# IanYeung/RealVSR

Measured on AMD Instinct MI355X. Metric: HR frames/sec (fwd+bwd) on 5-frame 180x320 LR windows, higher is better.
Workload: dtype f32 (bf16x3 GEMM); 1 GPU; EDVR-M nf64, 5-frame 180x320 LR windows, batch 8 per GPU, x4 output, VideoSRModel.optimize_parameters: fwd + LapPyr(ssim,cb) on Y + GWLoss on CbCr + bwd + Adam step; per_gpu_batch=8, global_batch=8, parallelism=sequence-dp1, gemm=bf16x3 (3-term bf16 split on v_mfma_f32_32x32x16_bf16, f32 accumulate), lf_term=ssim (restated IQA_pytorch.SSIM, parity unpinned)

## Files before the change

realvsr_amd/csrc/conv2_kernels.hip:

```cpp
#define RVSR_DEFINE_PACK
#include "conv_plan.h"

#include "bf16x3.h"

#ifdef RVSR_ABL5
constexpr int ABL5 = RVSR_ABL5;
#else
constexpr int ABL5 = 0;
#endif

#ifdef RVSR_TIMELINE
__device__ unsigned long long rvsr_dbg[512];
extern "C" int rvsr_debug_read(unsigned long long* out) { return (int)hipMemcpyFromSymbol(out, HIP_SYMBOL(rvsr_dbg), sizeof(unsigned long long) * 512); }
#define STAMP(i) do { if (blockIdx.x == 77 && tid == 0) rvsr_dbg[(i)] = __builtin_amdgcn_s_memtime(); } while (0)
#else
#define STAMP(i) do {} while (0)
#endif

template <int MT, int MODE>
__device__ __forceinline__ void conv2_epilogue(f32x16 (&acc)[MT][2], const ConvFwdParams& p, const float* bias_s, int b,
                                               int o0, int row0, int col, int hi) {
    const float neg = p.act == 0 ? 1.f : (p.act == 1 ? 0.f : p.slope);
    const bool col_ok = col < p.Wout;
    const size_t HW = (size_t)p.Hout * p.Wout;
#pragma unroll
    for (int n = 0; n < 2; ++n) {
        const int row = row0 + n;
        if (row >= p.Hout) continue;
        const size_t pix = (size_t)row * p.Wout + col;
#pragma unroll
        for (int m = 0; m < MT; ++m) {
            float resv[16];
            if (MODE == 1) {
#pragma unroll
                for (int r = 0; r < 16; ++r) {
                    const int o = o0 + m * 32 + 4 * hi + (r & 3) + 8 * (r >> 2);
                    const bool ok = col_ok && o < p.Co;
                    resv[r] = p.res[ok ? ((size_t)b * p.Co + o) * HW + pix : 0];
                }
            }
#pragma unroll
            for (int r = 0; r < 16; ++r) {
                const int ol = m * 32 + 4 * hi + (r & 3) + 8 * (r >> 2);
                const int o = o0 + ol;
                const bool ok = col_ok && o < p.Co;
                const int oc = ok ? o : 0;
                float v = acc[m][n][r] + bias_s[ol];
                v = v > 0.f ? v : v * neg;
                if (MODE == 3) {
                    const size_t idx = (((size_t)b * (p.Co >> 2) + (oc >> 2)) * (2 * p.Hout) + 2 * row + ((oc >> 1) & 1)) *
                                           (2 * p.Wout) + 2 * col + (oc & 1);
                    if (ok) p.out1[idx] = v;
                } else if (MODE == 2) {
                    const bool first = oc < p.Co1;
                    float* dst = first ? p.out1 : p.out2;
                    const size_t idx = ((size_t)b * (first ? p.Co1 : p.Co - p.Co1) + (first ? oc : oc - p.Co1)) * HW + pix;
                    if (ok) dst[idx] = v;
                } else {
                    if (MODE == 1) v += resv[r];
                    if (ok) p.out1[((size_t)b * p.Co + oc) * HW + pix] = v;
                }
            }
        }
    }
}

template <int MT, int MODE>
__device__ __forceinline__ void conv2_epilogue_v4(f32x16 (&acc)[MT][2], const ConvFwdParams& p, const float* bias_s, int b,
                                                  int o0, int row0, int x0, int lo, int hi) {
    const float neg = p.act == 0 ? 1.f : (p.act == 1 ? 0.f : p.slope);
    const int j = lo & 3, col4 = x0 + (lo & ~3);
    const bool col_ok = col4 < p.Wout;
    const unsigned HW = (unsigned)(p.Hout * p.Wout), HW4 = 4u * HW;
    const __amdgpu_buffer_rsrc_t out_rs = buf_view_2g(p.out1 + (size_t)b * p.Co * HW);
    const __amdgpu_buffer_rsrc_t res_rs = buf_view_2g(MODE == 1 ? p.res + (size_t)b * p.Co * HW : p.out1);
#pragma unroll
    for (int n = 0; n < 2; ++n) {
        const int row = row0 + n;
        if (row >= p.Hout) continue;
        const unsigned lane_off = 4u * ((unsigned)(4 * hi + j) * HW + (unsigned)row * p.Wout + col4);
#pragma unroll
        for (int m = 0; m < MT; ++m) {
            float4 resv[4];
            unsigned off[4];
#pragma unroll
            for (int rg = 0; rg < 4; ++rg) {
                const int ob = o0 + m * 32 + 8 * rg;
                off[rg] = col_ok && ob + 4 * hi + j < p.Co ? lane_off : 0x80000000u;
                if (MODE == 1) {
                    typedef float f32x4v __attribute__((ext_vector_type(4)));
                    const f32x4v q = __builtin_bit_cast(f32x4v, __builtin_amdgcn_raw_buffer_load_b128(res_rs, (int)(off[rg] + (unsigned)ob * HW4), 0, 0));
                    resv[rg] = make_float4(q.x, q.y, q.z, q.w);
                }
            }
#pragma unroll
            for (int rg = 0; rg < 4; ++rg) {
                float r0 = acc[m][n][4 * rg + 0], r1 = acc[m][n][4 * rg + 1], r2 = acc[m][n][4 * rg + 2], r3 = acc[m][n][4 * rg + 3];
                quad_transpose4(r0, r1, r2, r3, lo);
                const int ol = m * 32 + 8 * rg + 4 * hi + j;
                const float bb = bias_s[ol];
                float4 v = make_float4(r0 + bb, r1 + bb, r2 + bb, r3 + bb);
                v.x = v.x > 0.f ? v.x : v.x * neg; v.y = v.y > 0.f ? v.y : v.y * neg;
                v.z = v.z > 0.f ? v.z : v.z * neg; v.w = v.w > 0.f ? v.w : v.w * neg;
                if (MODE == 1) { v.x += resv[rg].x; v.y += resv[rg].y; v.z += resv[rg].z; v.w += resv[rg].w; }
                buf_store4(out_rs, off[rg] + (unsigned)(o0 + m * 32 + 8 * rg) * HW4, 0u, v);
            }
        }
    }
}

__device__ __forceinline__ void half_swap(float& a, float& b) {
    asm volatile("s_nop 1\n\tv_permlane32_swap_b32 %0, %1\n\ts_nop 0" : "+v"(a), "+v"(b));
}
template <int MT, int MODE>
__device__ __forceinline__ void conv2_epilogue_wide(f32x16 (&acc)[MT][2], const ConvFwdParams& p, const float* bias_s, int b,
                                                    int o0, int row, int x0, int lo, int hi) {
    if (row >= p.Hout) return;
    const float neg = (p.act == 0 || MODE == 4) ? 1.f : (p.act == 1 ? 0.f : p.slope);
    const int lane = 32 * hi + lo, jn = lane >> 4, Gn = lane & 15;
    const int src4 = 4 * (4 * Gn + jn);
    const int col4 = x0 + 4 * Gn;
    const bool col_ok = col4 < p.Wout;
    const unsigned HW = (unsigned)(p.Hout * p.Wout), HW4 = 4u * HW;
    const __amdgpu_buffer_rsrc_t out_rs = buf_view_2g(p.out1 + (size_t)b * p.Co * HW);
    const __amdgpu_buffer_rsrc_t res_rs = buf_view_2g(MODE == 1 || MODE == 4 ? p.res + (size_t)b * p.Co * HW : p.out1);
    const unsigned lane_off = 4u * ((unsigned)jn * HW + (unsigned)row * p.Wout + col4);
    const int j = lo & 3;
#pragma unroll
    for (int m = 0; m < MT; ++m) {
#pragma unroll
        for (int rg = 0; rg < 4; ++rg) {
            float4 resv[2];
            unsigned off[2];
#pragma unroll
            for (int s = 0; s < 2; ++s) {
                const int ob = o0 + m * 32 + 8 * rg + 4 * s;
                off[s] = col_ok && ob + jn < p.Co ? lane_off : 0x80000000u;
                if (MODE == 1 || MODE == 4) {
                    typedef float f32x4v __attribute__((ext_vector_type(4)));
                    const f32x4v q = __builtin_bit_cast(f32x4v, __builtin_amdgcn_raw_buffer_load_b128(res_rs, (int)(off[s] + (unsigned)ob * HW4), 0, 0));
                    resv[s] = make_float4(q.x, q.y, q.z, q.w);
                }
            }
            float r[2][4];
            const float bb = bias_s[m * 32 + 8 * rg + 4 * hi + j];
#pragma unroll
            for (int n = 0; n < 2; ++n) {
                r[n][0] = acc[m][n][4 * rg + 0]; r[n][1] = acc[m][n][4 * rg + 1]; r[n][2] = acc[m][n][4 * rg + 2]; r[n][3] = acc[m][n][4 * rg + 3];
                quad_transpose4(r[n][0], r[n][1], r[n][2], r[n][3], lo);
#pragma unroll
                for (int e = 0; e < 4; ++e) {
                    const float v = r[n][e] + bb;
                    r[n][e] = v > 0.f ? v : v * neg;
                }
            }
#pragma unroll
            for (int e = 0; e < 4; ++e) half_swap(r[0][e], r[1][e]);
#pragma unroll
            for (int s = 0; s < 2; ++s)
#pragma unroll
                for (int e = 0; e < 4; ++e)
                    r[s][e] = __builtin_bit_cast(float, __builtin_amdgcn_ds_bpermute(src4, __builtin_bit_cast(int, r[s][e])));
#pragma unroll
            for (int s = 0; s < 2; ++s) {
                float4 v = make_float4(r[s][0], r[s][1], r[s][2], r[s][3]);
                if (MODE == 1) { v.x += resv[s].x; v.y += resv[s].y; v.z += resv[s].z; v.w += resv[s].w; }
                if (MODE == 4) {
                    v.x *= resv[s].x > 0.f ? 1.f : p.slope; v.y *= resv[s].y > 0.f ? 1.f : p.slope;
                    v.z *= resv[s].z > 0.f ? 1.f : p.slope; v.w *= resv[s].w > 0.f ? 1.f : p.slope;
                }
                if (!(ABL5 & 2) || (m == 0 && rg == 0 && s == 0))
                buf_store4(out_rs, off[s] + (unsigned)(o0 + m * 32 + 8 * rg + 4 * s) * HW4, 0u, v);
            }
        }
    }
}

template <int KS, int STRIDE, int MT, int CCG, bool ACT_IN, int NW>
__global__ __launch_bounds__(NW * 64, 2) void conv_fwd2_kernel(const ConvFwdParams p) {
    constexpr int T = KS * KS, PAD = KS / 2, TH = 2 * NW, TW = 32, NTHR = NW * 64;
    constexpr int IH = (TH - 1) * STRIDE + KS, IW = (TW - 1) * STRIDE + KS;
    constexpr int MP = MT * 32, NOCT = 2 * CCG, NPOS = IH * IW;
    constexpr int WVEC = T * NOCT * MP;
    extern __shared__ __attribute__((aligned(16))) unsigned char smem_raw[];
    bf16x8* xs_hi = reinterpret_cast<bf16x8*>(smem_raw);
    bf16x8* xs_lo = xs_hi + NOCT * NPOS;
    bf16x8* ws_hi = xs_lo + NOCT * NPOS;
    bf16x8* ws_lo = ws_hi + WVEC;
    float* bias_s = reinterpret_cast<float*>(ws_lo + WVEC);
    const int tid = threadIdx.x, lane = tid & 63, wave = tid >> 6, lo = lane & 31, hi = lane >> 5;
    const TView& va = p.in.a;
    const TView& vb = p.in.b;
    const int C1 = va.C, Ctot = va.C + vb.C;
    const int nchunks = (Ctot + 16 * CCG - 1) / (16 * CCG);

    const unsigned nmb = (p.Co + MP - 1) / MP, nty = (p.Hout + TH - 1) / TH, ntx = (p.Wout + TW - 1) / TW;
    const unsigned items = ntx * nty * nmb * p.B;
    const unsigned xcd = blockIdx.x & 7, wq = blockIdx.x >> 3, nwq = (gridDim.x + 7 - xcd) >> 3;
    const unsigned q8 = items >> 3, r8 = items & 7;
    const unsigned range0 = xcd < r8 ? xcd * (q8 + 1) : r8 * (q8 + 1) + (xcd - r8) * q8;
    const unsigned range1 = range0 + q8 + (xcd < r8 ? 1 : 0);

    int x0 = 0, y0 = 0, mb = 0, b = 0;
    auto decode = [&](unsigned S) {
        const unsigned t = S % (p.ntx * nty);
        x0 = (int)(t % p.ntx) * TW;
        y0 = (int)(t / p.ntx) * TH;
        mb = (int)((S / (p.ntx * nty)) % nmb);
        b = (int)(S / (p.ntx * nty * nmb));
    };

    constexpr int NIT = (NOCT * NPOS + NTHR - 1) / NTHR;
    constexpr int NWV = (2 * WVEC + NTHR - 1) / NTHR;
    float vin[NIT][8];
    float ain[ACT_IN ? NIT : 1][8];
    int nvalid[NIT];

    __amdgpu_buffer_rsrc_t xa_rs = buf_view_2g(va.p), xb_rs = buf_view_2g(va.p), act_rs = buf_view_2g(va.p);
    auto tile_views = [&]() {
        if (va.mode != 0) return;
        const size_t hw = (size_t)va.Hs * va.Ws;
        xa_rs = buf_view_2g(va.p + (size_t)b * va.C * hw);
        if (vb.C) xb_rs = buf_view_2g(vb.p + (size_t)b * vb.C * hw);
        if (ACT_IN) act_rs = buf_view_2g(va.act + (size_t)b * va.C * hw);
    };
    auto issue_loads = [&](int chunk, int i_lo = 0, int i_hi = 1 << 20) {
        const int c0 = chunk * 16 * CCG;
#pragma unroll
        for (int i = 0; i < NIT; ++i) {
            if (i < i_lo || i >= i_hi) continue;
            const int it_raw = tid + i * NTHR;
            const bool live = it_raw < NOCT * NPOS;
            const int it = live ? it_raw : 0;
            const int oc = it / NPOS, pos = it - oc * NPOS;
            const int r = pos / IW, s = pos - r * IW;
            const int gy = y0 * STRIDE - PAD + r, gx = x0 * STRIDE - PAD + s;
            const int cb = c0 + oc * 8;
            const bool inb = live && gy >= 0 && gx >= 0 && gy < va.Hv && gx < va.Wv && cb < Ctot;
            const int gyc = gy < 0 ? 0 : (gy >= va.Hv ? va.Hv - 1 : gy), gxc = gx < 0 ? 0 : (gx >= va.Wv ? va.Wv - 1 : gx);
            if (va.mode == 0) {
                const bool second = c0 >= C1;
                const int Cb = second ? vb.C : va.C, cl0 = second ? c0 - C1 : c0;
                const unsigned hw4 = 4u * (unsigned)(va.Hs * va.Ws);
                const bool pos_ok = live && gy >= 0 && gx >= 0 && gy < va.Hv && gx < va.Wv;
                const unsigned vo = pos_ok ? 4u * (unsigned)(gy * va.Ws + gx) + (unsigned)(8 * oc) * hw4 : 0x80000000u;
                const int lane_nch = Cb - cl0 - 8 * oc;
                nvalid[i] = 8;
#pragma unroll
                for (int j = 0; j < 8; ++j) {
                    const unsigned vo_j = j < lane_nch ? vo : 0x80000000u;
                    const unsigned so = (unsigned)(cl0 + j) * hw4;
                    vin[i][j] = buf_load(second ? xb_rs : xa_rs, vo_j, so);
                    if (ACT_IN) ain[i][j] = buf_load(act_rs, vo_j, so);
                }
            } else {
                const size_t hw = (size_t)va.Hs * va.Ws;
                const int cbc = inb ? cb : 0;
                const size_t base = ((size_t)b * (va.C >> 2) + (cbc >> 2)) * hw + (size_t)(2 * gyc) * va.Ws + 2 * gxc;
                nvalid[i] = inb ? 8 : 0;
#pragma unroll
                for (int j = 0; j < 8; ++j) {
                    const size_t idx = base + (j >> 2) * hw + ((j >> 1) & 1) * va.Ws + (j & 1);
                    vin[i][j] = va.p[idx];
                    if (ACT_IN) ain[i][j] = va.act[idx];
                }
            }
        }
    };
    auto commit_inputs = [&](int i_lo = 0, int i_hi = 1 << 20) {
#pragma unroll
        for (int i = 0; i < NIT; ++i) {
            if (i < i_lo || i >= i_hi) continue;
            const int it = tid + i * NTHR;
            float v[8];
#pragma unroll
            for (int j = 0; j < 8; ++j) {
                float x = ACT_IN ? vin[i][j] * (ain[i][j] > 0.f ? 1.f : va.slope) : vin[i][j];
                v[j] = j < nvalid[i] ? x : 0.f;
            }
            bf16x8 h8, l8;
            split8(v, h8, l8);
            if (it < NOCT * NPOS) {
                xs_hi[it] = h8;
                xs_lo[it] = l8;
            }
        }
    };
    auto commit_to_lds = [&](int chunk, bool inputs_done = false) {
        const bf16x8* src = reinterpret_cast<const bf16x8*>(p.wpack) + ((size_t)mb * nchunks + chunk) * 2 * WVEC;
        constexpr int WB = MT >= 4 ? 3 : 9;
        constexpr bool OVERLAP = !ACT_IN && MT <= 2;
        if (!OVERLAP && !inputs_done) commit_inputs();
#pragma unroll
        for (int base = 0; base < NWV; base += WB) {
            bf16x8 wv[WB];
#pragma unroll
            for (int i = 0; i < WB; ++i) {
                const int e = tid + (base + i) * NTHR;
                wv[i] = src[(base + i < NWV && e < 2 * WVEC) ? e : 0];
            }
            if (OVERLAP && base == 0 && !inputs_done) commit_inputs();
#pragma unroll
            for (int i = 0; i < WB; ++i) {
                const int e = tid + (base + i) * NTHR;
                if (base + i < NWV && e < 2 * WVEC) ws_hi[e] = wv[i];
            }
        }
        if (chunk == 0 && tid < MP) {
            const int o = mb * MP + tid;
            bias_s[tid] = (p.bias != nullptr && o < p.Co) ? p.bias[o] : 0.f;
        }
    };

    constexpr bool PF = !ACT_IN && MT <= 2 && STRIDE == 1;
    unsigned S = range0 + wq;
    if (S < range1) {
        decode(S);
        tile_views();
        if (PF) issue_loads(0);
    }
    for (; S < range1; S += nwq) {
        f32x16 acc[MT][2];
#pragma unroll
        for (int m = 0; m < MT; ++m) {
            acc[m][0] = zero16();
            acc[m][1] = zero16();
        }
        const int cx0 = x0, cy0 = y0, cmb = mb, cb_ = b;
        STAMP(0);
        for (int chunk = 0; chunk < nchunks; ++chunk) {
            constexpr int NB = 3;
            if (!PF && STRIDE == 2) {
#pragma unroll
                for (int i0 = 0; i0 < NIT; i0 += NB) {
                    issue_loads(chunk, i0, i0 + NB);
                    commit_inputs(i0, i0 + NB);
                }
                commit_to_lds(chunk, true);
            } else {
                if (!PF) issue_loads(chunk);
                commit_to_lds(chunk);
            }
            STAMP(1 + chunk * 5);
            __syncthreads();
            STAMP(2 + chunk * 5);
            if (PF && chunk + 1 < nchunks) issue_loads(chunk + 1);
            STAMP(3 + chunk * 5);
#pragma unroll
            for (int tap = 0; tap < T; ++tap) {
                const int dy = tap / KS, dx = tap % KS;
#pragma unroll
                for (int g = 0; g < CCG; ++g) {
                    const int oc = 2 * g + hi;
                    bf16x8 ah[MT], al[MT], bh[2], bl[2];
#pragma unroll
                    for (int m = 0; m < MT; ++m) {
                        ah[m] = ws_hi[(tap * NOCT + oc) * MP + m * 32 + lo];
                        al[m] = ws_lo[(tap * NOCT + oc) * MP + m * 32 + lo];
                    }
#pragma unroll
                    for (int n = 0; n < 2; ++n) {
                        const int idx = (oc * IH + (wave * 2 + n) * STRIDE + dy) * IW + lo * STRIDE + dx;
                        bh[n] = xs_hi[idx];
                        bl[n] = xs_lo[idx];
                    }
#pragma unroll
                    for (int m = 0; m < MT; ++m)
#pragma unroll
                        for (int n = 0; n < 2; ++n) acc[m][n] = mfma_bf16(ah[m], bh[n], acc[m][n]);
#pragma unroll
                    for (int m = 0; m < MT; ++m)
#pragma unroll
                        for (int n = 0; n < 2; ++n) acc[m][n] = mfma_bf16(ah[m], bl[n], acc[m][n]);
#pragma unroll
                    for (int m = 0; m < MT; ++m)
#pragma unroll
                        for (int n = 0; n < 2; ++n) acc[m][n] = mfma_bf16(al[m], bh[n], acc[m][n]);
                }
            }
            STAMP(4 + chunk * 5);
            __syncthreads();
            STAMP(5 + chunk * 5);
        }
        if (p.ps)
            conv2_epilogue<MT, 3>(acc, p, bias_s, cb_, cmb * MP, cy0 + wave * 2, cx0 + lo, hi);
        else if (p.out2 != nullptr)
            conv2_epilogue<MT, 2>(acc, p, bias_s, cb_, cmb * MP, cy0 + wave * 2, cx0 + lo, hi);
        else if (p.res != nullptr) {
            if (p.vec4) conv2_epilogue_v4<MT, 1>(acc, p, bias_s, cb_, cmb * MP, cy0 + wave * 2, cx0, lo, hi);
            else conv2_epilogue<MT, 1>(acc, p, bias_s, cb_, cmb * MP, cy0 + wave * 2, cx0 + lo, hi);
        } else {
            if (p.vec4) conv2_epilogue_v4<MT, 0>(acc, p, bias_s, cb_, cmb * MP, cy0 + wave * 2, cx0, lo, hi);
            else conv2_epilogue<MT, 0>(acc, p, bias_s, cb_, cmb * MP, cy0 + wave * 2, cx0 + lo, hi);
        }
        STAMP(30);
        if (S + nwq < range1) {
            decode(S + nwq);
            tile_views();
            if (PF) issue_loads(0);
        }
        STAMP(31);
        __syncthreads();
    }
}

template <int MT, bool ACT_IN, int VEC, bool WIDE = false, int NT = 3>
__global__ __launch_bounds__(512, 2) void conv_fwd5_kernel(const ConvFwdParams p) {
    constexpr int KS = 3, T = 9, PAD = 1, NW = 8, TH = WIDE ? NW : 2 * NW, TW = WIDE ? 64 : 32, NTHR = NW * 64;
    constexpr int IH = TH + KS - 1, IW = TW + KS - 1;
    constexpr int MP = MT * 32, NOCT = 2, NPOS = IH * IW, NX = NOCT * NPOS;
    constexpr int WVEC = T * NOCT * MP;
    extern __shared__ __attribute__((aligned(16))) unsigned char smem_raw[];
    bf16x8* xs_base = reinterpret_cast<bf16x8*>(smem_raw);
    bf16x8* ws_base = xs_base + 2 * 2 * NX;
    float* bias_base = reinterpret_cast<float*>(ws_base + 2 * 2 * WVEC);
    bf16x8* const sink = reinterpret_cast<bf16x8*>(bias_base + 4 * MP);
    const int tid = threadIdx.x, lane = tid & 63, wave = tid >> 6, lo = lane & 31, hi = lane >> 5;
    const TView& va = p.in.a;
    const TView& vb = p.in.b;
    const int C1 = va.C, Ctot = va.C + vb.C;
    const int nchunks = (Ctot + 15) / 16;

    const unsigned nmb = (p.Co + MP - 1) / MP, nty = (p.Hout + TH - 1) / TH, ntx = (p.Wout + TW - 1) / TW;
    const unsigned items = ntx * nty * nmb * p.B;
    const unsigned xcd = blockIdx.x & 7, wq = blockIdx.x >> 3, nwq = (gridDim.x + 7 - xcd) >> 3;
    const unsigned q8 = items >> 3, r8 = items & 7;
    const unsigned range0 = xcd < r8 ? xcd * (q8 + 1) : r8 * (q8 + 1) + (xcd - r8) * q8;
    const unsigned range1 = range0 + q8 + (xcd < r8 ? 1 : 0);
    const unsigned S0 = range0 + wq;
    if (S0 >= range1) return;
    const int ntile = (int)((range1 - S0 + nwq - 1) / nwq);
    const int Q = ntile * nchunks;

    struct Tile { int x0, y0, mb, b; };
    auto tile_of = [&](int k) {
        const unsigned S = S0 + (unsigned)k * nwq;
        Tile t;
        const unsigned u = S % (ntx * nty);
        t.x0 = (int)(u % ntx) * TW;
        t.y0 = (int)(u / ntx) * TH;
        t.mb = (int)((S / (ntx * nty)) % nmb);
        t.b = (int)(S / (ntx * nty * nmb));
        return t;
    };

    constexpr int NG = TW / 4 + 2;
    __amdgpu_buffer_rsrc_t w_rs = buf_view_2g(p.wpack), xa_rs = buf_view_2g(va.p), xb_rs = buf_view_2g(va.p), act_rs = buf_view_2g(va.p);
    constexpr int NIT = VEC ? 1 : (NX + NTHR - 1) / NTHR;
    constexpr int WPARTS = NT >= 3 ? 2 : 1;
    constexpr int NWV = (WPARTS * WVEC + NTHR - 1) / NTHR;
    constexpr int NV = VEC ? 4 : 1;
    int it_oc[NIT], it_sp[NIT], it_dst[NIT];
    bool it_pos_ok[NIT];
    auto item_geom = [&](const Tile& t) {
#pragma unroll
        for (int i = 0; i < NIT; ++i) {
            if (VEC) {
                const bool live = tid < NOCT * IH * NG;
                const int it = live ? tid : 0;
                const int oc = it / (IH * NG), rem = it - oc * (IH * NG);
                const int r = rem / NG, g = rem - r * NG;
                const int gy = t.y0 - PAD + r, gx = t.x0 - 4 + 4 * g;
                it_oc[i] = oc;
                it_pos_ok[i] = live && gy >= 0 && gy < va.Hv && gx >= 0 && gx < va.Wv;
                if (VEC == 3)
                    it_sp[i] = it_pos_ok[i] && !(gy & 1) && (gy >> 1) < va.Hs ? 4 * ((gy >> 1) * va.Ws + (gx >> 1)) : (int)0x80000000;
                else
                    it_sp[i] = it_pos_ok[i] ? (VEC == 2 ? 8 * (gy * va.Ws + gx) : 4 * (gy * va.Ws + gx)) : (int)0x80000000;
                it_dst[i] = live ? (oc * IH + r) * IW + 4 * g - 3 : -100;
            } else {
                const int it_raw = tid + i * NTHR;
                const bool live = it_raw < NX;
                const int it = live ? it_raw : 0;
                const int oc = it / NPOS, pos = it - oc * NPOS;
                const int r = pos / IW, s = pos - r * IW;
                const int gy = t.y0 - PAD + r, gx = t.x0 - PAD + s;
                it_oc[i] = oc;
                bool ok = live && gy >= 0 && gx >= 0 && gy < va.Hv && gx < va.Wv;
                const int gyc = gy < 0 ? 0 : (gy >= va.Hv ? va.Hv - 1 : gy), gxc = gx < 0 ? 0 : (gx >= va.Wv ? va.Wv - 1 : gx);
                if (va.mode == 1) {
                    const int ys = gyc >> 1, xs = gxc >> 1;
                    ok = ok && !((gyc | gxc) & 1) && ys < va.Hs && xs < va.Ws;
                    it_sp[i] = (ys < va.Hs ? ys : 0) * va.Ws + (xs < va.Ws ? xs : 0);
                } else {
                    it_sp[i] = va.mode == 0 ? gyc * va.Ws + gxc : (2 * gyc) * va.Ws + 2 * gxc;
                }
                it_pos_ok[i] = ok;
                it_dst[i] = live ? it : -100;
            }
        }
    };
    float vin[NIT][8][NV];
    float ain[ACT_IN ? NIT : 1][8][NV];
    int nvalid[NIT];
    bf16x8 wv[NWV];
    typedef unsigned u32x4 __attribute__((ext_vector_type(4)));
    typedef float f32x4v __attribute__((ext_vector_type(4)));
    auto issue_loads = [&](const Tile& t, int chunk, int wsel, int xsel) {
        if (VEC) {
            const unsigned wbase = (unsigned)(((size_t)t.mb * nchunks + chunk) * 2 * WVEC) * 16u;
#pragma unroll
            for (int i = 0; i < NWV; ++i) {
                if (wsel >= 0 && wsel != i) continue;
                const int e = tid + i * NTHR;
                const unsigned vo = e < WPARTS * WVEC ? (unsigned)tid * 16u : 0x80000000u;
                const u32x4 w = __builtin_amdgcn_raw_buffer_load_b128(w_rs, (int)vo, (int)(wbase + (unsigned)i * NTHR * 16u), 0);
                wv[i] = __builtin_bit_cast(bf16x8, w);
            }
            if (xsel >= 8) return;
            const int c0 = chunk * 16;
            const bool second = c0 >= C1;
            const int Cb = second ? vb.C : va.C, cl0 = second ? c0 - C1 : c0;
            const unsigned hw4 = 4u * (unsigned)(va.Hs * va.Ws);
            const int lane_nch = Cb - cl0 - 8 * it_oc[0];
            nvalid[0] = 8;
            if (VEC == 2) {
                const unsigned row4 = 4u * (unsigned)va.Ws, pl4 = row4 * (unsigned)va.Hs;
                const unsigned vo = (unsigned)it_sp[0] + (unsigned)(2 * it_oc[0]) * pl4;
                const unsigned vo_l = lane_nch > 0 ? vo : 0x80000000u;
#pragma unroll
                for (int l = 0; l < 8; ++l) {
                    const int csl = l >> 2, sy = (l >> 1) & 1, half = l & 1;
                    if (xsel >= 0 && csl != xsel) continue;
                    const unsigned so = (unsigned)((cl0 >> 2) + csl) * pl4 + (unsigned)sy * row4 + 16u * half;
                    const f32x4v q = __builtin_bit_cast(f32x4v, __builtin_amdgcn_raw_buffer_load_b128(xa_rs, (int)vo_l, (int)so, 0));
                    const int j0 = 4 * csl + 2 * sy, e0 = (2 * half) & (NV - 1), e1 = (2 * half + 1) & (NV - 1);
                    vin[0][j0][e0] = q.x; vin[0][j0 + 1][e0] = q.y; vin[0][j0][e1] = q.z; vin[0][j0 + 1][e1] = q.w;
                    if (ACT_IN) {
                        const f32x4v a4 = __builtin_bit_cast(f32x4v, __builtin_amdgcn_raw_buffer_load_b128(act_rs, (int)vo_l, (int)so, 0));
                        ain[0][j0][e0] = a4.x; ain[0][j0 + 1][e0] = a4.y; ain[0][j0][e1] = a4.z; ain[0][j0 + 1][e1] = a4.w;
                    }
                }
                return;
            }
            const unsigned vo = (unsigned)it_sp[0] + (unsigned)(8 * it_oc[0]) * hw4;
            if (VEC == 3) {
                typedef float f32x2v __attribute__((ext_vector_type(2)));
#pragma unroll
                for (int j = 0; j < 8; ++j) {
                    if (xsel >= 0 && (j >> 2) != xsel) continue;
                    const unsigned so = (unsigned)(cl0 + j) * hw4;
                    const unsigned vo_j = j < lane_nch ? vo : 0x80000000u;
                    const f32x2v q = __builtin_bit_cast(f32x2v, __builtin_amdgcn_raw_buffer_load_b64(xa_rs, (int)vo_j, (int)so, 0));
                    vin[0][j][0] = q.x; vin[0][j][NV > 2 ? 2 : 0] = q.y; vin[0][j][NV > 1 ? 1 : 0] = 0.f; vin[0][j][NV > 3 ? 3 : 0] = 0.f;
                    if (ACT_IN) {
                        const f32x2v a2 = __builtin_bit_cast(f32x2v, __builtin_amdgcn_raw_buffer_load_b64(act_rs, (int)vo_j, (int)so, 0));
                        ain[0][j][0] = a2.x; ain[0][j][NV > 2 ? 2 : 0] = a2.y; ain[0][j][NV > 1 ? 1 : 0] = 1.f; ain[0][j][NV > 3 ? 3 : 0] = 1.f;
                    }
                }
                return;
            }
#pragma unroll
// ... 158 lines not shown
    f32x16 acc[MT][2];
#pragma unroll
    for (int m = 0; m < MT; ++m) {
        acc[m][0] = zero16();
        acc[m][1] = zero16();
    }
    for (int q = 0; q < Q; ++q) {
        STAMP(1 + (q & 7) * 3);
        const int buf = q & 1;
        const bf16x8* xs_hi = xs_base + buf * 2 * NX;
        const bf16x8* xs_lo = xs_hi + NX;
        const bf16x8* ws_hi = ws_base + buf * 2 * WVEC;
        const bf16x8* ws_lo = ws_hi + WVEC;
        constexpr bool pub = true;
        bf16x8 ah[2][MT], al[2][MT], bh[2][2], bl[2][2];
        auto fetch = [&](int tap, int slot) {
            const int dy = tap / KS, dx = tap % KS;
#pragma unroll
            for (int m = 0; m < MT; ++m) {
                ah[slot][m] = ws_hi[(tap * NOCT + hi) * MP + m * 32 + lo];
                if (NT >= 3) al[slot][m] = ws_lo[(tap * NOCT + hi) * MP + m * 32 + lo];
            }
#pragma unroll
            for (int n = 0; n < 2; ++n) {
                const int idx = WIDE ? (hi * IH + wave + dy) * IW + lo + 32 * n + dx : (hi * IH + wave * 2 + n + dy) * IW + lo + dx;
                bh[slot][n] = xs_hi[idx];
                if (NT >= 2) bl[slot][n] = xs_lo[idx];
            }
        };
        fetch(0, 0);
#pragma unroll
        for (int tap = 0; tap < T; ++tap) {
            const int sl = tap & 1;
#ifdef RVSR_TIMELINE
            if (blockIdx.x == 77 && lane == 0 && q == Q - 6) rvsr_dbg[300 + wave * 12 + tap] = __builtin_amdgcn_s_memtime();
#endif
            if (NT == 4) {
                typedef _Float16 f16x8m __attribute__((ext_vector_type(8)));
                typedef int i32x4m __attribute__((ext_vector_type(4)));
                typedef int i32x8m __attribute__((ext_vector_type(8)));
                const int sa = hi ? 127 - 12 : 127, sb = hi ? 127 : 127 - 12;
                if (tap & 1) {
#pragma unroll
                    for (int m = 0; m < MT; ++m)
#pragma unroll
                        for (int n = 0; n < 2; ++n) {
                            const i32x8m pa = __builtin_shufflevector(__builtin_bit_cast(i32x4m, al[sl ^ 1][m]), __builtin_bit_cast(i32x4m, al[sl][m]), 0, 1, 2, 3, 4, 5, 6, 7);
                            const i32x8m pb = __builtin_shufflevector(__builtin_bit_cast(i32x4m, bl[sl ^ 1][n]), __builtin_bit_cast(i32x4m, bl[sl][n]), 0, 1, 2, 3, 4, 5, 6, 7);
                            acc[m][n] = __builtin_amdgcn_mfma_scale_f32_32x32x64_f8f6f4(pa, pb, acc[m][n], 0, 0, 0, sa, 0, sb);
                        }
                }
                if (tap + 1 < T) fetch(tap + 1, sl ^ 1);
#pragma unroll
                for (int m = 0; m < MT; ++m)
#pragma unroll
                    for (int n = 0; n < 2; ++n)
                        acc[m][n] = __builtin_amdgcn_mfma_f32_32x32x16_f16(__builtin_bit_cast(f16x8m, ah[sl][m]), __builtin_bit_cast(f16x8m, bh[sl][n]), acc[m][n], 0, 0, 0);
                if (tap == T - 1) {
                    const i32x4m z = {0, 0, 0, 0};
#pragma unroll
                    for (int m = 0; m < MT; ++m)
#pragma unroll
                        for (int n = 0; n < 2; ++n) {
                            const i32x8m pa = __builtin_shufflevector(__builtin_bit_cast(i32x4m, al[sl][m]), z, 0, 1, 2, 3, 4, 5, 6, 7);
                            const i32x8m pb = __builtin_shufflevector(__builtin_bit_cast(i32x4m, bl[sl][n]), __builtin_bit_cast(i32x4m, bl[sl][n]), 0, 1, 2, 3, 4, 5, 6, 7);
                            acc[m][n] = __builtin_amdgcn_mfma_scale_f32_32x32x64_f8f6f4(pa, pb, acc[m][n], 0, 0, 0, sa, 0, sb);
                        }
                }
            } else {
            if (tap + 1 < ((ABL5 & 1) ? 2 : T)) fetch(tap + 1, sl ^ 1);
#pragma unroll
            for (int m = 0; m < MT; ++m)
#pragma unroll
                for (int n = 0; n < 2; ++n) acc[m][n] = mfma_bf16(ah[sl][m], bh[sl][n], acc[m][n]);
            if (NT >= 2) {
#pragma unroll
                for (int m = 0; m < MT; ++m)
#pragma unroll
                    for (int n = 0; n < 2; ++n) acc[m][n] = mfma_bf16(ah[sl][m], bl[sl][n], acc[m][n]);
            }
            if (NT >= 3) {
#pragma unroll
                for (int m = 0; m < MT; ++m)
#pragma unroll
                    for (int n = 0; n < 2; ++n) acc[m][n] = mfma_bf16(al[sl][m], bh[sl][n], acc[m][n]);
            }
            }
            if (tap < 4) {
                if (pub) commit(buf ^ 1, NWV, tap);
            } else {
                if (pub) commit(buf ^ 1, tap - 4, 8);
                if (tap == 4) stage_tile(q + 2, k_nx2, c_nx2);
                issue_stage(q + 2, c_nx2, tap - 4, (ABL5 & 4) ? 8 : VEC ? (tap < 6 ? tap - 4 : 8) : (tap - 4 < NIT ? tap - 4 : 8));
            }
            __builtin_amdgcn_sched_barrier(0);
        }
        STAMP(2 + (q & 7) * 3);
#ifdef RVSR_TIMELINE
        if (blockIdx.x == 77 && lane == 0 && q == Q - 3) rvsr_dbg[70 + wave] = __builtin_amdgcn_s_memtime();
        if (blockIdx.x == 77 && lane == 0 && q == Q - 4) rvsr_dbg[90 + wave] = __builtin_amdgcn_s_memtime();
        if (blockIdx.x == 77 && lane == 0 && q == Q - 6) rvsr_dbg[300 + wave * 12 + 9] = __builtin_amdgcn_s_memtime();
#endif
        const int k = k_cur;
        const bool last_chunk = c_cur == nchunks - 1;
        if (++c_cur == nchunks) { c_cur = 0; ++k_cur; }
        if (++c_nx2 == nchunks) { c_nx2 = 0; ++k_nx2; }
        if (last_chunk) {
            const Tile cur = tile_of(k);
            const float* bias_s = bias_base + (k & 3) * MP;
            if (WIDE) {
                if (p.act == 3) conv2_epilogue_wide<MT, 4>(acc, p, bias_s, cur.b, cur.mb * MP, cur.y0 + wave, cur.x0, lo, hi);
                else if (p.res != nullptr) conv2_epilogue_wide<MT, 1>(acc, p, bias_s, cur.b, cur.mb * MP, cur.y0 + wave, cur.x0, lo, hi);
                else conv2_epilogue_wide<MT, 0>(acc, p, bias_s, cur.b, cur.mb * MP, cur.y0 + wave, cur.x0, lo, hi);
            } else if (p.ps)
                conv2_epilogue<MT, 3>(acc, p, bias_s, cur.b, cur.mb * MP, cur.y0 + wave * 2, cur.x0 + lo, hi);
            else if (p.out2 != nullptr)
                conv2_epilogue<MT, 2>(acc, p, bias_s, cur.b, cur.mb * MP, cur.y0 + wave * 2, cur.x0 + lo, hi);
            else if (p.res != nullptr) {
                if (p.vec4) conv2_epilogue_v4<MT, 1>(acc, p, bias_s, cur.b, cur.mb * MP, cur.y0 + wave * 2, cur.x0, lo, hi);
                else conv2_epilogue<MT, 1>(acc, p, bias_s, cur.b, cur.mb * MP, cur.y0 + wave * 2, cur.x0 + lo, hi);
            } else {
                if (p.vec4) conv2_epilogue_v4<MT, 0>(acc, p, bias_s, cur.b, cur.mb * MP, cur.y0 + wave * 2, cur.x0, lo, hi);
                else conv2_epilogue<MT, 0>(acc, p, bias_s, cur.b, cur.mb * MP, cur.y0 + wave * 2, cur.x0 + lo, hi);
            }
#pragma unroll
            for (int m = 0; m < MT; ++m) {
                acc[m][0] = zero16();
                acc[m][1] = zero16();
            }
        }
        __syncthreads();
        STAMP(3 + (q & 7) * 3);
#ifdef RVSR_TIMELINE
        if (blockIdx.x == 77 && lane == 0 && q == Q - 4) rvsr_dbg[80 + wave] = __builtin_amdgcn_s_memtime();
        if (blockIdx.x == 77 && lane == 0 && q == Q - 6) rvsr_dbg[300 + wave * 12 + 10] = __builtin_amdgcn_s_memtime();
        if (blockIdx.x == 77 && lane == 0 && q == Q - 7) rvsr_dbg[300 + wave * 12 + 11] = __builtin_amdgcn_s_memtime();
#endif
    }
    STAMP(61);
#ifdef RVSR_TIMELINE
    if (blockIdx.x == 77 && tid == 0) rvsr_dbg[62] = (unsigned long long)Q;
#endif
}


size_t rvsr_conv_fwd2_workspace_bytes(int ksize, int Co, int Ctot) {
    int mt, ccg, nchunks, nmb;
    conv_fwd2_geom(ksize, Co, Ctot, mt, ccg, nchunks, nmb);
    return (size_t)nmb * nchunks * 2 * (ksize * ksize) * (2 * ccg) * (mt * 32) * 16;
}

typedef void (*ConvFwdKernel)(const ConvFwdParams);

static ConvFwdKernel fwd2_kernel(int ksize, int stride, const ConvFwdPlan& q) {
#define ROW(KS, STRIDE, MT, CCG) \
    if (ksize == KS && stride == STRIDE && q.mt == MT) return q.act_in ? conv_fwd2_kernel<KS, STRIDE, MT, CCG, true, 4> : conv_fwd2_kernel<KS, STRIDE, MT, CCG, false, 4>
    ROW(3, 2, 1, 1);
    ROW(3, 2, 2, 1);
    ROW(5, 1, 1, 1);
    ROW(5, 2, 1, 1);
    ROW(1, 1, 1, 2);
    ROW(1, 1, 2, 2);
#undef ROW
    return nullptr;
}

static ConvFwdKernel fwd5_kernel(const ConvFwdPlan& q) {
#define ROW(MT, VEC, WIDE, NT) \
    if (q.mt == MT && q.vec == VEC && q.wide == WIDE && q.nt == NT) return q.act_in ? conv_fwd5_kernel<MT, true, VEC, WIDE, NT> : conv_fwd5_kernel<MT, false, VEC, WIDE, NT>
    ROW(2, 1, true, 3);
    ROW(2, 1, true, 2);
    ROW(2, 1, true, 1);
    ROW(2, 1, false, 3);
    ROW(2, 1, false, 2);
    ROW(2, 1, false, 1);
    ROW(2, 2, false, 3);
    ROW(2, 2, false, 2);
    ROW(2, 2, false, 1);
    ROW(2, 3, false, 3);
    ROW(2, 3, false, 2);
    ROW(2, 3, false, 1);
    ROW(2, 0, false, 3);
    ROW(1, 0, false, 3);
    ROW(1, 1, false, 3);
    ROW(1, 2, false, 3);
    ROW(1, 3, false, 3);
#undef ROW
    if (q.mt == 2 && q.vec == 1 && q.nt == 4 && !q.act_in) return q.wide ? conv_fwd5_kernel<2, false, 1, true, 4> : conv_fwd5_kernel<2, false, 1, false, 4>;
    return nullptr;
}

int rvsr_launch_conv_fwd2(ConvFwdParams p, const ConvFwdPlan& q, int ksize, int stride, void* workspace, size_t workspace_bytes, hipStream_t st) {
    const int Ctot = p.in.a.C + p.in.b.C, T = ksize * ksize;
    int mt, ccg, nchunks, nmb;
    conv_fwd2_geom(ksize, p.Co, Ctot, mt, ccg, nchunks, nmb);
    const size_t need = rvsr_conv_fwd2_workspace_bytes(ksize, p.Co, Ctot);
    if (!workspace || workspace_bytes < need) FAIL(RVSR_ERR_WORKSPACE, "conv2d: workspace %zu B < %zu B", workspace_bytes, need);
    const bool five = q.family == CONV_FWD5;
    const ConvFwdKernel k = five ? fwd5_kernel(q) : fwd2_kernel(ksize, stride, q);
    if (!k) FAIL(RVSR_ERR_LAUNCH, "conv2d: no %s instantiation for this plan", five ? "conv_fwd5" : "conv_fwd2");
    if (!p.prepacked) {
        const size_t total = (size_t)nmb * nchunks * T * (2 * ccg) * (mt * 32);
        hipLaunchKernelGGL(pack_weights_kernel, dim3((unsigned)((total + 255) / 256)), dim3(256), 0, st, p.w, (bf16x8*)workspace, p.Co,
                           Ctot, T, mt * 32, ccg, nchunks, nmb, p.w_mode | (p.fmt ? 0x100 : 0));
    }
    p.wpack = workspace;
    p.vec4 = q.vec4;
    return rvsr_conv_launch(five ? "conv_fwd5" : "conv_fwd2", k, dim3(q.gx), five ? 512 : 256, q.lds, st, p);
}

extern "C" size_t rvsr_conv2d_pack_weights(const float* weight, int C_in, int Co, int ksize, int w_mode, void* out, size_t out_bytes,
                                           long long* desc, void* stream) {
    int mt, ccg, nchunks, nmb;
    if (ksize != 1 && ksize != 3 && ksize != 5) return 0;
    conv_fwd2_geom(ksize, Co, C_in, mt, ccg, nchunks, nmb);
    const size_t need = rvsr_conv_fwd2_workspace_bytes(ksize, Co, C_in);
    if (!weight || !out || out_bytes < need) return 0;
    if ((w_mode & 4) && !conv_f16fp8_ok(ksize, 1, mt, w_mode & 1)) return 0;
    const int fmtflag = (w_mode & 4) ? 0x100 : 0;
    const int T = ksize * ksize;
    const size_t total = (size_t)nmb * nchunks * T * (2 * ccg) * (mt * 32);
    hipLaunchKernelGGL(pack_weights_kernel, dim3((unsigned)((total + 255) / 256)), dim3(256), 0, (hipStream_t)stream, weight, (bf16x8*)out, Co,
                       C_in, T, mt * 32, ccg, nchunks, nmb, (w_mode & 1) | fmtflag);
    if (desc) {
        desc[0] = (long long)(uintptr_t)weight; desc[1] = (long long)(uintptr_t)out;
        desc[2] = Co; desc[3] = C_in; desc[4] = T; desc[5] = mt * 32; desc[6] = ccg; desc[7] = nchunks; desc[8] = nmb; desc[9] = (w_mode & 1) | fmtflag;
    }
    return need;
}
extern "C" int rvsr_pack_weights_batched(const void* descs, int n, void* stream) {
    if (n <= 0) return RVSR_OK;
    if (!descs) FAIL(RVSR_ERR_BAD_ARG, "pack_weights_batched: null table");
    static_assert(sizeof(PackDesc) == 48, "PackDesc layout is part of the C ABI (two pointers + eight ints)");
    hipLaunchKernelGGL(pack_weights_batched_kernel, dim3(16, (unsigned)n), dim3(256), 0, (hipStream_t)stream, (const PackDesc*)descs);
    hipError_t e = hipGetLastError();
    if (e != hipSuccess) FAIL(RVSR_ERR_LAUNCH, "pack_weights_batched launch: %s", hipGetErrorString(e));
    return RVSR_OK;
}

#define WG2_THREADS 512
#define WG2_GP 272
#define WG2_XP 496

typedef unsigned int u32x4 __attribute__((ext_vector_type(4)));

__device__ __forceinline__ bf16x8 as_bf16x8(u32x4 v) { return __builtin_bit_cast(bf16x8, v); }

template <int SHIFT>
__device__ __forceinline__ bf16x8 take8(u32x4 a, u32x4 b) {
    u32x4 r;
    if (SHIFT == 4) {
        r[0] = a[2]; r[1] = a[3]; r[2] = b[0]; r[3] = b[1];
    } else if (SHIFT == 3) {
        r[0] = __builtin_amdgcn_alignbit(a[2], a[1], 16);
        r[1] = __builtin_amdgcn_alignbit(a[3], a[2], 16);
        r[2] = __builtin_amdgcn_alignbit(b[0], a[3], 16);
        r[3] = __builtin_amdgcn_alignbit(b[1], b[0], 16);
    } else {
        r[0] = __builtin_amdgcn_alignbit(a[3], a[2], 16);
        r[1] = __builtin_amdgcn_alignbit(b[0], a[3], 16);
        r[2] = __builtin_amdgcn_alignbit(b[1], b[0], 16);
        r[3] = __builtin_amdgcn_alignbit(b[2], b[1], 16);
    }
    return as_bf16x8(r);
}

template <int DXMASK, int NT>
__device__ __forceinline__ void wg2_row(const unsigned char* xs_hi, const unsigned char* xs_lo, int xoff, bf16x8 ah,
                                        bf16x8 al, f32x16* acc) {
    const u32x4 h0 = *reinterpret_cast<const u32x4*>(xs_hi + xoff), h1 = *reinterpret_cast<const u32x4*>(xs_hi + xoff + 16);
    constexpr int N = ((DXMASK >> 0) & 1) + ((DXMASK >> 1) & 1) + ((DXMASK >> 2) & 1);
    bf16x8 bh[3], bl[3];
    int t = 0;
    if (DXMASK & 1) { bh[t] = take8<3>(h0, h1); ++t; }
    if (DXMASK & 2) { bh[t] = take8<4>(h0, h1); ++t; }
    if (DXMASK & 4) { bh[t] = take8<5>(h0, h1); ++t; }
    if (NT >= 2) {
        const u32x4 l0 = *reinterpret_cast<const u32x4*>(xs_lo + xoff), l1 = *reinterpret_cast<const u32x4*>(xs_lo + xoff + 16);
        t = 0;
        if (DXMASK & 1) { bl[t] = take8<3>(l0, l1); ++t; }
        if (DXMASK & 2) { bl[t] = take8<4>(l0, l1); ++t; }
        if (DXMASK & 4) { bl[t] = take8<5>(l0, l1); ++t; }
    }
#pragma unroll
    for (int i = 0; i < N; ++i) acc[i] = mfma_bf16(ah, bh[i], acc[i]);
    if (NT >= 2) {
#pragma unroll
        for (int i = 0; i < N; ++i) acc[i] = mfma_bf16(ah, bl[i], acc[i]);
    }
    if (NT >= 3) {
#pragma unroll
        for (int i = 0; i < N; ++i) acc[i] = mfma_bf16(al, bh[i], acc[i]);
    }
}

#ifndef WGRAD2_RING
#define WGRAD2_RING 0
#endif
template <bool ACT, int GMODE, int NT = 3>
__global__ __launch_bounds__(WG2_THREADS, 2) void conv_wgrad2_kernel(const ConvWgradParams p) {
    extern __shared__ __attribute__((aligned(16))) unsigned char smem_raw[];
    unsigned char* gs_hi = smem_raw;
    unsigned char* gs_lo = gs_hi + 64 * WG2_GP;
    unsigned char* xs_hi = gs_lo + 64 * WG2_GP;
    unsigned char* xs_lo = xs_hi + 64 * WG2_XP;
    float* bsum = reinterpret_cast<float*>(xs_lo + 64 * WG2_XP);
    const int tid = threadIdx.x, lane = tid & 63, wave = tid >> 6, lo = lane & 31, hi = lane >> 5;
    const int mb = blockIdx.y, c0 = blockIdx.z * 64;
    const int Ctot = p.x.a.C + p.x.b.C, C1 = p.x.a.C;
    const int H = p.x.a.Hs, W = p.x.a.Ws;
    const int m = wave & 1, chalf = (wave >> 1) & 1, second = wave >> 2;
    const bool m_live = (mb * 64 + m * 32) < p.Co;
    const bool do_bias = p.bpart != nullptr && blockIdx.z == 0;

    f32x16 acc[5];
#pragma unroll
    for (int i = 0; i < 5; ++i) acc[i] = zero16();
    if (tid < 64) bsum[tid] = 0.f;
    __syncthreads();

    constexpr int NGI = 2;
    constexpr int NGV = GMODE == 0 ? 2 : 4;
    constexpr int NXI = 4;
    float4 gv[NGI][NGV], sv[ACT ? NGI : 1][NGV], xv[NXI][2];
    float bacc[NGI] = {0.f, 0.f};

    constexpr unsigned OOB = 0x80000000u;
    unsigned g_vo[NGI], x_vo[NXI];
    int g_row[NGI], g_gx8[NGI], g_o[NGI], g_lds[NGI];
#pragma unroll
    for (int i = 0; i < NGI; ++i) {
        const int it = tid + i * WG2_THREADS;
        const int q = it & 3, row = (it >> 2) & 3, ol = it >> 4;
        g_row[i] = row;
        g_gx8[i] = 8 * q;
        g_o[i] = mb * 64 + ol;
        g_lds[i] = ol * WG2_GP + row * 64 + q * 16;
        const int o = g_o[i];
        g_vo[i] = o >= p.Co ? OOB
                : 4u * (GMODE == 0 ? (unsigned)((o * H + row) * W + 8 * q)
                                   : (unsigned)((((o >> 2) * 2 * H) + 2 * row + ((o >> 1) & 1)) * (2 * W) + 16 * q));
    }
    const bool sec = c0 >= C1;
    int x_row[NXI], x_gx[NXI], x_lds[NXI];
#pragma unroll
    for (int i = 0; i < NXI; ++i) {
        const int it_raw = tid + i * WG2_THREADS;
        const bool live = it_raw < 64 * 30;
        const int it = live ? it_raw : 0;
        const int cl = it / 30, rem = it - cl * 30;
        const int row = rem / 5, q = rem - row * 5;
        const int c = c0 + cl;
        x_row[i] = row - 1;
        x_gx[i] = 8 * q - 4;
        x_lds[i] = live ? cl * WG2_XP + q * 16 : -1;
        x_vo[i] = live && c < Ctot ? 4u * (unsigned)(((sec ? c - C1 : c) * H + row) * W + 8 * q) : OOB;
    }
    const size_t img_g = (size_t)p.Co * H * W;
    const size_t img_x1 = (size_t)C1 * H * W, img_x2 = (size_t)(Ctot - C1) * H * W;

    struct TilePos { int b, y0, x0; bool fresh; };
// ... 660 lines not shown
```

Before: 83.62 HR frames/s.

## Add 16-byte staging, 8-wave M split, and cross-tile prefetch to conv_fwd2

Gives the 1x1 conv a 16-byte vectorized input staging path with an XOR-swizzled LDS column layout, and puts the M-block index innermost so consecutive work items reuse the same input tile. The 3x3 stride-2 MT=2 case without input activation now runs with 8 waves, which split the two M tiles between them. Prefetch of the next work item's first chunk now overlaps the current tile's last-chunk compute instead of waiting until after the epilogue. These changes target global load instruction count, LDS bank conflicts and load latency exposed between tiles, at the cost of more kernel variants, higher register pressure and new alignment preconditions. TH is fixed at 8, so the tile shape no longer follows NW.

```diff
diff --git a/realvsr_amd/csrc/conv2_kernels.hip b/realvsr_amd/csrc/conv2_kernels.hip
--- a/realvsr_amd/csrc/conv2_kernels.hip
+++ b/realvsr_amd/csrc/conv2_kernels.hip
@@ -176,9 +176,12 @@
     }
 }
 
-template <int KS, int STRIDE, int MT, int CCG, bool ACT_IN, int NW>
+template <int KS, int STRIDE, int MT, int CCG, bool ACT_IN, int NW, bool V16 = false>
 __global__ __launch_bounds__(NW * 64, 2) void conv_fwd2_kernel(const ConvFwdParams p) {
-    constexpr int T = KS * KS, PAD = KS / 2, TH = 2 * NW, TW = 32, NTHR = NW * 64;
+    constexpr int T = KS * KS, PAD = KS / 2, TH = 8, TW = 32, NTHR = NW * 64;
+    constexpr int MS = NW / 4, MTW = MT / MS;
+    static_assert((NW == 4 || NW == 8) && MTW * MS == MT, "4 waves, or 8 waves over two M tiles");
+    static_assert(!V16 || (KS == 1 && STRIDE == 1 && CCG == 2 && NW == 4), "16-byte staging: the 1x1 tile, one octet per wave");
     constexpr int IH = (TH - 1) * STRIDE + KS, IW = (TW - 1) * STRIDE + KS;
     constexpr int MP = MT * 32, NOCT = 2 * CCG, NPOS = IH * IW;
     constexpr int WVEC = T * NOCT * MP;
@@ -189,6 +192,7 @@
     bf16x8* ws_lo = ws_hi + WVEC;
     float* bias_s = reinterpret_cast<float*>(ws_lo + WVEC);
     const int tid = threadIdx.x, lane = tid & 63, wave = tid >> 6, lo = lane & 31, hi = lane >> 5;
+    const int wrow = wave & 3, wm = (wave >> 2) * MTW;
     const TView& va = p.in.a;
     const TView& vb = p.in.b;
     const int C1 = va.C, Ctot = va.C + vb.C;
@@ -202,13 +206,15 @@
     const unsigned range1 = range0 + q8 + (xcd < r8 ? 1 : 0);
 
     int x0 = 0, y0 = 0, mb = 0, b = 0;
+    constexpr bool MB_INNER = KS == 1;
     auto decode = [&](unsigned S) {
-        const unsigned t = S % (p.ntx * nty);
+        const unsigned t = MB_INNER ? (S / nmb) % (p.ntx * nty) : S % (p.ntx * nty);
         x0 = (int)(t % p.ntx) * TW;
         y0 = (int)(t / p.ntx) * TH;
-        mb = (int)((S / (p.ntx * nty)) % nmb);
+        mb = (int)(MB_INNER ? S % nmb : (S / (p.ntx * nty)) % nmb);
         b = (int)(S / (p.ntx * nty * nmb));
     };
+    auto xs_col = [](int x) { return V16 ? (x ^ ((x >> 3) & 3)) : x; };
 
     constexpr int NIT = (NOCT * NPOS + NTHR - 1) / NTHR;
     constexpr int NWV = (2 * WVEC + NTHR - 1) / NTHR;
@@ -238,7 +244,30 @@
             const int cb = c0 + oc * 8;
             const bool inb = live && gy >= 0 && gx >= 0 && gy < va.Hv && gx < va.Wv && cb < Ctot;
             const int gyc = gy < 0 ? 0 : (gy >= va.Hv ? va.Hv - 1 : gy), gxc = gx < 0 ? 0 : (gx >= va.Wv ? va.Wv - 1 : gx);
-            if (va.mode == 0) {
+            if (V16) {
+                if (i != 0) continue;
+                typedef float f32x4v __attribute__((ext_vector_type(4)));
+                const int oc4 = tid >> 6, r4 = (tid >> 3) & 7, q4 = tid & 7;
+                const int gy4 = y0 + r4, gx4 = x0 + 4 * q4;
+                const bool second = c0 >= C1;
+                const int Cb = second ? vb.C : va.C, cl0 = second ? c0 - C1 : c0;
+                const unsigned hw4 = 4u * (unsigned)(va.Hs * va.Ws);
+                const unsigned vo = gy4 < va.Hv && gx4 < va.Wv ? 4u * (unsigned)(gy4 * va.Ws + gx4) + (unsigned)(8 * oc4) * hw4 : 0x80000000u;
+                const int lane_nch = Cb - cl0 - 8 * oc4;
+#pragma unroll
+                for (int e = 0; e < NIT; ++e) nvalid[e] = 8;
+#pragma unroll
+                for (int j = 0; j < 8; ++j) {
+                    const unsigned vo_j = j < lane_nch ? vo : 0x80000000u;
+                    const unsigned so = (unsigned)(cl0 + j) * hw4;
+                    const f32x4v v4 = __builtin_bit_cast(f32x4v, __builtin_amdgcn_raw_buffer_load_b128(second ? xb_rs : xa_rs, (int)vo_j, (int)so, 0));
+                    vin[0][j] = v4.x; vin[1 % NIT][j] = v4.y; vin[2 % NIT][j] = v4.z; vin[3 % NIT][j] = v4.w;
+                    if (ACT_IN) {
+                        const f32x4v a4 = __builtin_bit_cast(f32x4v, __builtin_amdgcn_raw_buffer_load_b128(act_rs, (int)vo_j, (int)so, 0));
+                        ain[0][j] = a4.x; ain[1 % NIT][j] = a4.y; ain[2 % NIT][j] = a4.z; ain[3 % NIT][j] = a4.w;
+                    }
+                }
+            } else if (va.mode == 0) {
                 const bool second = c0 >= C1;
                 const int Cb = second ? vb.C : va.C, cl0 = second ? c0 - C1 : c0;
                 const unsigned hw4 = 4u * (unsigned)(va.Hs * va.Ws);
@@ -271,7 +300,7 @@
 #pragma unroll
         for (int i = 0; i < NIT; ++i) {
             if (i < i_lo || i >= i_hi) continue;
-            const int it = tid + i * NTHR;
+            const int it = V16 ? (tid >> 3) * 32 + xs_col(4 * (tid & 7) + i) : tid + i * NTHR;
             float v[8];
 #pragma unroll
             for (int j = 0; j < 8; ++j) {
@@ -289,7 +318,7 @@
     auto commit_to_lds = [&](int chunk, bool inputs_done = false) {
         const bf16x8* src = reinterpret_cast<const bf16x8*>(p.wpack) + ((size_t)mb * nchunks + chunk) * 2 * WVEC;
         constexpr int WB = MT >= 4 ? 3 : 9;
-        constexpr bool OVERLAP = !ACT_IN && MT <= 2;
+        constexpr bool OVERLAP = (!ACT_IN || V16) && MT <= 2;
         if (!OVERLAP && !inputs_done) commit_inputs();
 #pragma unroll
         for (int base = 0; base < NWV; base += WB) {
@@ -312,7 +341,7 @@
         }
     };
 
-    constexpr bool PF = !ACT_IN && MT <= 2 && STRIDE == 1;
+    constexpr bool PF = MT <= 2 && (STRIDE == 1 ? (!ACT_IN || V16) : (NW == 8 && !ACT_IN));
     unsigned S = range0 + wq;
     if (S < range1) {
         decode(S);
@@ -320,9 +349,9 @@
         if (PF) issue_loads(0);
     }
     for (; S < range1; S += nwq) {
-        f32x16 acc[MT][2];
-#pragma unroll
-        for (int m = 0; m < MT; ++m) {
+        f32x16 acc[MTW][2];
+#pragma unroll
+        for (int m = 0; m < MTW; ++m) {
             acc[m][0] = zero16();
             acc[m][1] = zero16();
         }
@@ -344,7 +373,15 @@
             STAMP(1 + chunk * 5);
             __syncthreads();
             STAMP(2 + chunk * 5);
-            if (PF && chunk + 1 < nchunks) issue_loads(chunk + 1);
+            if (PF) {
+                int next = chunk + 1;
+                if (next == nchunks) {
+                    next = 0;
+                    decode(S + nwq < range1 ? S + nwq : S);
+                    tile_views();
+                }
+                issue_loads(next);
+            }
             STAMP(3 + chunk * 5);
 #pragma unroll
             for (int tap = 0; tap < T; ++tap) {
@@ -352,28 +389,28 @@
 #pragma unroll
                 for (int g = 0; g < CCG; ++g) {
                     const int oc = 2 * g + hi;
-                    bf16x8 ah[MT], al[MT], bh[2], bl[2];
-#pragma unroll
-                    for (int m = 0; m < MT; ++m) {
-                        ah[m] = ws_hi[(tap * NOCT + oc) * MP + m * 32 + lo];
-                        al[m] = ws_lo[(tap * NOCT + oc) * MP + m * 32 + lo];
+                    bf16x8 ah[MTW], al[MTW], bh[2], bl[2];
+#pragma unroll
+                    for (int m = 0; m < MTW; ++m) {
+                        ah[m] = ws_hi[(tap * NOCT + oc) * MP + (wm + m) * 32 + lo];
+                        al[m] = ws_lo[(tap * NOCT + oc) * MP + (wm + m) * 32 + lo];
                     }
 #pragma unroll
                     for (int n = 0; n < 2; ++n) {
-                        const int idx = (oc * IH + (wave * 2 + n) * STRIDE + dy) * IW + lo * STRIDE + dx;
+                        const int idx = (oc * IH + (wrow * 2 + n) * STRIDE + dy) * IW + xs_col(lo * STRIDE + dx);
                         bh[n] = xs_hi[idx];
                         bl[n] = xs_lo[idx];
                     }
 #pragma unroll
-                    for (int m = 0; m < MT; ++m)
+                    for (int m = 0; m < MTW; ++m)
 #pragma unroll
                         for (int n = 0; n < 2; ++n) acc[m][n] = mfma_bf16(ah[m], bh[n], acc[m][n]);
 #pragma unroll
-                    for (int m = 0; m < MT; ++m)
+                    for (int m = 0; m < MTW; ++m)
 #pragma unroll
                         for (int n = 0; n < 2; ++n) acc[m][n] = mfma_bf16(ah[m], bl[n], acc[m][n]);
 #pragma unroll
-                    for (int m = 0; m < MT; ++m)
+                    for (int m = 0; m < MTW; ++m)
 #pragma unroll
                         for (int n = 0; n < 2; ++n) acc[m][n] = mfma_bf16(al[m], bh[n], acc[m][n]);
                 }
@@ -382,22 +419,23 @@
             __syncthreads();
             STAMP(5 + chunk * 5);
         }
+        const int wo0 = cmb * MP + wm * 32, wy0 = cy0 + wrow * 2;
+        const float* wbias = bias_s + wm * 32;
         if (p.ps)
-            conv2_epilogue<MT, 3>(acc, p, bias_s, cb_, cmb * MP, cy0 + wave * 2, cx0 + lo, hi);
+            conv2_epilogue<MTW, 3>(acc, p, wbias, cb_, wo0, wy0, cx0 + lo, hi);
         else if (p.out2 != nullptr)
-            conv2_epilogue<MT, 2>(acc, p, bias_s, cb_, cmb * MP, cy0 + wave * 2, cx0 + lo, hi);
+            conv2_epilogue<MTW, 2>(acc, p, wbias, cb_, wo0, wy0, cx0 + lo, hi);
         else if (p.res != nullptr) {
-            if (p.vec4) conv2_epilogue_v4<MT, 1>(acc, p, bias_s, cb_, cmb * MP, cy0 + wave * 2, cx0, lo, hi);
-            else conv2_epilogue<MT, 1>(acc, p, bias_s, cb_, cmb * MP, cy0 + wave * 2, cx0 + lo, hi);
+            if (p.vec4) conv2_epilogue_v4<MTW, 1>(acc, p, wbias, cb_, wo0, wy0, cx0, lo, hi);
+            else conv2_epilogue<MTW, 1>(acc, p, wbias, cb_, wo0, wy0, cx0 + lo, hi);
         } else {
-            if (p.vec4) conv2_epilogue_v4<MT, 0>(acc, p, bias_s, cb_, cmb * MP, cy0 + wave * 2, cx0, lo, hi);
-            else conv2_epilogue<MT, 0>(acc, p, bias_s, cb_, cmb * MP, cy0 + wave * 2, cx0 + lo, hi);
+            if (p.vec4) conv2_epilogue_v4<MTW, 0>(acc, p, wbias, cb_, wo0, wy0, cx0, lo, hi);
+            else conv2_epilogue<MTW, 0>(acc, p, wbias, cb_, wo0, wy0, cx0 + lo, hi);
         }
         STAMP(30);
-        if (S + nwq < range1) {
+        if (!PF && S + nwq < range1) {
             decode(S + nwq);
             tile_views();
-            if (PF) issue_loads(0);
         }
         STAMP(31);
         __syncthreads();
@@ -862,11 +900,21 @@
 
 typedef void (*ConvFwdKernel)(const ConvFwdParams);
 
-static ConvFwdKernel fwd2_kernel(int ksize, int stride, const ConvFwdPlan& q) {
+static ConvFwdKernel fwd2_kernel(int ksize, int stride, const ConvFwdPlan& q, bool v16, unsigned& threads) {
+    threads = 256;
+    if (ksize == 3 && stride == 2 && q.mt == 2) {
+        if (q.act_in) return conv_fwd2_kernel<3, 2, 2, 1, true, 4>;
+        threads = 512;
+        return conv_fwd2_kernel<3, 2, 2, 1, false, 8>;
+    }
 #define ROW(KS, STRIDE, MT, CCG) \
     if (ksize == KS && stride == STRIDE && q.mt == MT) return q.act_in ? conv_fwd2_kernel<KS, STRIDE, MT, CCG, true, 4> : conv_fwd2_kernel<KS, STRIDE, MT, CCG, false, 4>
+#define ROW16(MT) \
+    if (ksize == 1 && stride == 1 && q.mt == MT && v16) return q.act_in ? conv_fwd2_kernel<1, 1, MT, 2, true, 4, true> : conv_fwd2_kernel<1, 1, MT, 2, false, 4, true>
+    ROW16(1);
+    ROW16(2);
+#undef ROW16
     ROW(3, 2, 1, 1);
-    ROW(3, 2, 2, 1);
     ROW(5, 1, 1, 1);
     ROW(5, 2, 1, 1);
     ROW(1, 1, 1, 2);
@@ -907,7 +955,11 @@
     const size_t need = rvsr_conv_fwd2_workspace_bytes(ksize, p.Co, Ctot);
     if (!workspace || workspace_bytes < need) FAIL(RVSR_ERR_WORKSPACE, "conv2d: workspace %zu B < %zu B", workspace_bytes, need);
     const bool five = q.family == CONV_FWD5;
-    const ConvFwdKernel k = five ? fwd5_kernel(q) : fwd2_kernel(ksize, stride, q);
+    const TView& va = p.in.a;
+    const bool v16 = !five && ksize == 1 && stride == 1 && va.mode == 0 && va.Ws % 4 == 0 && va.Wv == va.Ws &&
+                     conv_al16(va.p, va.act, p.in.b.p);
+    unsigned threads = 512;
+    const ConvFwdKernel k = five ? fwd5_kernel(q) : fwd2_kernel(ksize, stride, q, v16, threads);
     if (!k) FAIL(RVSR_ERR_LAUNCH, "conv2d: no %s instantiation for this plan", five ? "conv_fwd5" : "conv_fwd2");
     if (!p.prepacked) {
         const size_t total = (size_t)nmb * nchunks * T * (2 * ccg) * (mt * 32);
@@ -916,7 +968,7 @@
     }
     p.wpack = workspace;
     p.vec4 = q.vec4;
-    return rvsr_conv_launch(five ? "conv_fwd5" : "conv_fwd2", k, dim3(q.gx), five ? 512 : 256, q.lds, st, p);
+    return rvsr_conv_launch(five ? "conv_fwd5" : "conv_fwd2", k, dim3(q.gx), threads, q.lds, st, p);
 }
 
 extern "C" size_t rvsr_conv2d_pack_weights(const float* weight, int C_in, int Co, int ksize, int w_mode, void* out, size_t out_bytes,
```

Measured after the change: 84.15 HR frames/s, median of 6. About the same (+0.6%).
